# facebookresearch/vggsfm

Measured on NVIDIA H100. Metric: BA iterations/sec, higher is better.
Workload: dtype f64

## Files before the change

### vggsfm_b200/_lib.py

```python
from __future__ import annotations

import ctypes
import os

_HERE = os.path.dirname(os.path.abspath(__file__))
LIB_PATH = os.path.join(_HERE, "libvggsfm_b200.so")

EXPORTS = [
    "vgg_last_error", "vgg_version",
    "vgg_ba_default_options", "vgg_ba_dims", "vgg_ba_workspace_bytes", "vgg_ba_camrec_len",
    "vgg_ba_build_blocks", "vgg_ba_schur", "vgg_cholesky_lower", "vgg_ba_solve",
    "vgg_ba_reduced_system_doubles", "vgg_ba_fabric_doubles", "vgg_ba_solve_fabric",
    "vgg_ba_default_linear_solver", "vgg_ba_workspace_bytes_iterative", "vgg_ba_solve_iterative",
    "vgg_pose_default_options", "vgg_pose_refinement", "vgg_pnp_workspace_bytes", "vgg_absolute_pose_estimation", "vgg_syrk_ozaki_workspace_bytes", "vgg_syrk_ozaki",
    "vgg_tri_workspace_bytes", "vgg_triangulate_tracks", "vgg_triangulate_by_pair", "vgg_filter_points3d",
    "vgg_project_points", "vgg_normalize_tracks", "vgg_undistort_simple_radial",
    "vgg_corr_pyramid_bytes", "vgg_corr_build_pyramid", "vgg_corr_sample", "vgg_sample_features4d",
    "vgg_corr_tc_supported", "vgg_corr_tc_bytes", "vgg_corr_tc_build", "vgg_corr_tc_sample",
    "vgg_twoview_workspace_bytes", "vgg_estimate_fundamental", "vgg_relative_pose_from_fundamental",
    "vgg_fundamental_inliers", "vgg_msac_fundamental_workspace_bytes", "vgg_estimate_fundamental_msac",
    "vgg_depth_sparse_samples", "vgg_depth_median", "vgg_depth_ransac_workspace_bytes", "vgg_depth_ransac_max_chunk",
    "vgg_depth_ransac_begin", "vgg_depth_ransac_chunk", "vgg_depth_ransac_finish", "vgg_depth_tile_pixels",
    "vgg_depth_apply", "vgg_depth_unproject",
]


DEV_EXPORTS = ["vgg_dev_blocks_timing", "vgg_dev_blocks_last_ms", "vgg_dev_chol128_probe", "vgg_dev_syrk_f64", "vgg_dev_syrk_f64_band", "vgg_dev_trsv_probe", "vgg_dev_cholesky_band",
               "vgg_dev_last_band_hint", "vgg_dev_msac_trace", "vgg_dev_relative_pose_counts",
               "vgg_dev_build_blocks_band", "vgg_dev_schur_build", "vgg_dev_syrk_work_list", "vgg_dev_pcg_probe"]


class BAProblem(ctypes.Structure):
    _fields_ = [
        ("S", ctypes.c_int32), ("N", ctypes.c_int32),
        ("camera_model", ctypes.c_int32), ("intr_mode", ctypes.c_int32),
        ("uv", ctypes.c_void_p), ("mask", ctypes.c_void_p),
        ("param_const", ctypes.c_void_p), ("point_const", ctypes.c_void_p),
        ("poses", ctypes.c_void_p), ("intr", ctypes.c_void_p), ("points", ctypes.c_void_p),
        ("loss_function_type", ctypes.c_int32), ("loss_function_scale", ctypes.c_double),
    ]


class BAOptions(ctypes.Structure):
    _fields_ = [
        ("max_num_iterations", ctypes.c_int32),
        ("max_num_consecutive_invalid_steps", ctypes.c_int32),
        ("jacobi_scaling", ctypes.c_int32),
        ("reserved", ctypes.c_int32),
        ("function_tolerance", ctypes.c_double),
        ("gradient_tolerance", ctypes.c_double),
        ("parameter_tolerance", ctypes.c_double),
        ("initial_trust_region_radius", ctypes.c_double),
        ("max_trust_region_radius", ctypes.c_double),
        ("min_trust_region_radius", ctypes.c_double),
        ("min_relative_decrease", ctypes.c_double),
        ("min_lm_diagonal", ctypes.c_double),
        ("max_lm_diagonal", ctypes.c_double),
    ]


class BALinearSolver(ctypes.Structure):
    _fields_ = [
        ("type", ctypes.c_int32), ("min_linear_solver_iterations", ctypes.c_int32),
        ("max_linear_solver_iterations", ctypes.c_int32), ("eta", ctypes.c_double),
    ]


class BASummary(ctypes.Structure):
    _fields_ = [
        ("iterations", ctypes.c_int32), ("successful", ctypes.c_int32),
        ("termination", ctypes.c_int32), ("reserved", ctypes.c_int32),
        ("initial_cost", ctypes.c_double), ("final_cost", ctypes.c_double),
        ("final_radius", ctypes.c_double), ("device_ms", ctypes.c_double),
        ("kernel_launches", ctypes.c_int64),
    ]


class BAFabric(ctypes.Structure):
    _fields_ = [("ar_local", ctypes.c_void_p), ("ar_multicast", ctypes.c_void_p), ("ar_doubles", ctypes.c_size_t),
                ("world", ctypes.c_int32), ("rank", ctypes.c_int32), ("peer_base", ctypes.c_void_p * 8),
                ("total_doubles", ctypes.c_size_t)]


class PoseOptions(ctypes.Structure):
    _fields_ = [
        ("max_num_iterations", ctypes.c_int32),
        ("max_num_consecutive_invalid_steps", ctypes.c_int32),
        ("min_inliers", ctypes.c_int32),
        ("reserved", ctypes.c_int32),
        ("function_tolerance", ctypes.c_double),
        ("gradient_tolerance", ctypes.c_double),
        ("parameter_tolerance", ctypes.c_double),
        ("initial_trust_region_radius", ctypes.c_double),
        ("max_trust_region_radius", ctypes.c_double),
        ("min_trust_region_radius", ctypes.c_double),
        ("min_relative_decrease", ctypes.c_double),
        ("min_lm_diagonal", ctypes.c_double),
        ("max_lm_diagonal", ctypes.c_double),
        ("loss_function_scale", ctypes.c_double),
        ("max_reproj_error", ctypes.c_double),
    ]


ALLREDUCE_FN = ctypes.CFUNCTYPE(ctypes.c_int, ctypes.c_void_p, ctypes.c_void_p, ctypes.c_size_t,
                                ctypes.c_int, ctypes.c_void_p)

_lib = None


class NativeLibraryMissing(RuntimeError):
    pass


def lib() -> ctypes.CDLL:
    global _lib
    if _lib is not None:
        return _lib
    if not os.path.exists(LIB_PATH):
        raise NativeLibraryMissing(
            f"{LIB_PATH} not found: build it with `python -c 'import __graft_entry__ as g; g.build()'` "
            "or `make`. vggsfm_b200 has no CPU/PyTorch fallback.")
    L = ctypes.CDLL(LIB_PATH, mode=ctypes.RTLD_GLOBAL)
    L.vgg_last_error.restype = ctypes.c_char_p
    L.vgg_version.restype = ctypes.c_int
    L.vgg_ba_default_options.argtypes = [ctypes.POINTER(BAOptions)]
    L.vgg_ba_default_options.restype = None
    L.vgg_ba_dims.argtypes = [ctypes.c_int, ctypes.c_int, ctypes.POINTER(ctypes.c_int), ctypes.POINTER(ctypes.c_int)]
    L.vgg_ba_workspace_bytes.argtypes = [ctypes.c_int, ctypes.c_int, ctypes.c_int, ctypes.c_int,
                                         ctypes.POINTER(ctypes.c_size_t)]
    L.vgg_ba_camrec_len.argtypes = [ctypes.c_int, ctypes.c_int]
    L.vgg_ba_build_blocks.argtypes = [ctypes.POINTER(BAProblem)] + [ctypes.c_void_p] * 6 + [ctypes.c_int, ctypes.c_void_p]
    L.vgg_ba_schur.argtypes = ([ctypes.POINTER(BAProblem)] + [ctypes.c_void_p] * 5 +
                               [ctypes.c_double] * 3 + [ctypes.c_void_p, ctypes.c_size_t, ctypes.c_void_p,
                                                        ctypes.c_void_p, ctypes.POINTER(ctypes.c_int), ctypes.c_void_p])
    L.vgg_ba_solve.argtypes = [ctypes.POINTER(BAProblem), ctypes.POINTER(BAOptions), ctypes.c_void_p, ctypes.c_size_t,
                               ALLREDUCE_FN, ctypes.c_void_p, ctypes.POINTER(BASummary), ctypes.c_void_p,
                               ctypes.c_void_p]
    vp, ci, cd, cs = ctypes.c_void_p, ctypes.c_int, ctypes.c_double, ctypes.c_size_t
    L.vgg_ba_reduced_system_doubles.argtypes = [ci, ci, ci, ctypes.POINTER(cs)]
    L.vgg_ba_fabric_doubles.argtypes = [ci, ci, ci, ctypes.POINTER(cs)]
    L.vgg_ba_solve_fabric.argtypes = [ctypes.POINTER(BAProblem), ctypes.POINTER(BAOptions), vp, cs, ALLREDUCE_FN, vp,
                                      ctypes.POINTER(BAFabric), ctypes.POINTER(BASummary), vp, vp]
    L.vgg_ba_default_linear_solver.argtypes = [ctypes.POINTER(BALinearSolver)]
    L.vgg_ba_default_linear_solver.restype = None
    L.vgg_ba_workspace_bytes_iterative.argtypes = [ci, ci, ci, ci, ctypes.POINTER(cs)]
    L.vgg_ba_solve_iterative.argtypes = [ctypes.POINTER(BAProblem), ctypes.POINTER(BAOptions),
                                         ctypes.POINTER(BALinearSolver), vp, cs, ctypes.POINTER(BASummary), vp, vp, vp]
    L.vgg_dev_pcg_probe.argtypes = [ctypes.POINTER(BAProblem)] + [vp] * 6 + [cd] * 3 + [vp, vp, cs] + [vp] * 5
    L.vgg_pose_default_options.argtypes = [ctypes.POINTER(PoseOptions)]
    L.vgg_pose_default_options.restype = None
    L.vgg_pose_refinement.argtypes = [ci, ci, ci, vp, vp, vp, vp, vp, vp, ctypes.POINTER(PoseOptions), vp, vp, vp, vp]
    L.vgg_pnp_workspace_bytes.argtypes = [ci, ci, ctypes.POINTER(cs)]
    L.vgg_absolute_pose_estimation.argtypes = [ci, ci, ci, vp, vp, vp, vp, vp, vp, ci, ci, cd, vp, vp, vp, vp, vp, cs, vp]
    L.vgg_syrk_ozaki_workspace_bytes.argtypes = [ci, ci, ci, ctypes.POINTER(cs)]
    L.vgg_dev_blocks_timing.argtypes = [ci]
    L.vgg_dev_blocks_last_ms.argtypes = [ctypes.POINTER(cd)]
    L.vgg_dev_chol128_probe.argtypes = [ci, vp, vp, vp]
    L.vgg_dev_syrk_f64.argtypes = [ci, ci, vp, vp, vp]
    L.vgg_dev_syrk_f64_band.argtypes = L.vgg_dev_syrk_f64.argtypes + [vp, ci]
    L.vgg_dev_trsv_probe.argtypes = [ci, ci, vp, vp, cs, vp, vp]
    L.vgg_dev_last_band_hint.argtypes = [vp, vp, vp, vp, vp]
    L.vgg_dev_build_blocks_band.argtypes = L.vgg_ba_build_blocks.argtypes[:-1] + [vp, ci, vp]
    L.vgg_dev_schur_build.argtypes = [ctypes.POINTER(BAProblem)] + [vp] * 5 + [cd] * 3 + [ci, ci, vp, cs] + [vp] * 8
    L.vgg_dev_syrk_work_list.argtypes = [ci, ci, vp, ci, ci, vp, ci, ctypes.POINTER(ci)]
    L.vgg_syrk_ozaki.argtypes = [ci, ci, vp, vp, ci, vp, cs, vp]
    L.vgg_cholesky_lower.argtypes = [ci, ci, vp, vp, cs, ctypes.POINTER(ci), vp]
    L.vgg_dev_cholesky_band.argtypes = L.vgg_cholesky_lower.argtypes + [vp, ci, ci]
    L.vgg_tri_workspace_bytes.argtypes = [ci, ci, ci, ci, ctypes.POINTER(cs)]
    L.vgg_triangulate_tracks.argtypes = [ci, ci, vp, vp, vp, vp, vp, ci, ci, cd, cd, vp, vp, vp, vp, cs, vp]
    L.vgg_triangulate_by_pair.argtypes = [ci, ci, vp, vp, vp, vp, vp, vp, cs, vp]
    L.vgg_filter_points3d.argtypes = [ci, ci, vp, vp, ci, vp, vp, vp, cd, cd, ci, cd, vp, vp, vp, cs, vp]
    L.vgg_project_points.argtypes = [ci, ci, vp, vp, vp, vp, vp, vp, vp]
    L.vgg_normalize_tracks.argtypes = [ci, ci, vp, vp, vp, ci, vp, vp]
    L.vgg_undistort_simple_radial.argtypes = [ci, ci, vp, vp, ci, cd, cd, vp, ctypes.POINTER(ci), vp, cs, vp]
    L.vgg_corr_pyramid_bytes.argtypes = [ci, ci, ci, ci, ci, ci, ctypes.POINTER(cs), ctypes.POINTER(cs)]
    L.vgg_corr_build_pyramid.argtypes = [ci, ci, ci, ci, ci, vp, ci, vp, vp, vp]
    L.vgg_sample_features4d.argtypes = [ci, ci, ci, ci, ci, vp, vp, vp, vp]
    L.vgg_corr_sample.argtypes = [ci, ci, ci, ci, ci, ci, ci, vp, ci, vp, vp, ci, vp, vp]
    L.vgg_corr_tc_supported.argtypes = [ci, ci, ci, ci, ci]
    L.vgg_corr_tc_bytes.argtypes = [ci, ci, ci, ci, ci, ci, ctypes.POINTER(cs), ctypes.POINTER(cs)]
    L.vgg_corr_tc_build.argtypes = [ci, ci, ci, ci, ci, vp, vp, vp]
    L.vgg_corr_tc_sample.argtypes = [ci, ci, ci, ci, ci, ci, ci, vp, vp, vp, vp, vp, vp]
    L.vgg_twoview_workspace_bytes.argtypes = [ci, ci, ci, ci, ctypes.POINTER(cs)]
    L.vgg_estimate_fundamental.argtypes = [ci, ci, vp, vp, ci, vp, vp, ci, ci, cd, ci, ci, vp, vp, vp, vp, vp, cs, vp]
    L.vgg_fundamental_inliers.argtypes = [ci, ci, vp, vp, ci, vp, cd, ci, vp, vp]
    L.vgg_relative_pose_from_fundamental.argtypes = [ci, ci, vp, vp, ci, vp, cd, cd, vp, vp, vp, vp]
    L.vgg_dev_relative_pose_counts.argtypes = [ci, ci, vp, vp, ci, vp, cd, cd, vp, vp, vp, vp, vp]
    cu64 = ctypes.c_ulonglong
    L.vgg_msac_fundamental_workspace_bytes.argtypes = [ci, ci, ci, ci, ctypes.POINTER(cs)]
    L.vgg_estimate_fundamental_msac.argtypes = [ci, ci, vp, vp, ci, vp, cd, ci, ci, cu64, vp, vp, vp, vp, vp, cs, vp]
    L.vgg_dev_msac_trace.argtypes = [ci, ci, ci, ci, vp, ci, vp, vp, vp]
    i64 = ctypes.c_int64
    L.vgg_depth_sparse_samples.argtypes = [ci, vp, vp, cd, cd, vp, vp, vp, vp, vp, vp, vp]
    L.vgg_depth_median.argtypes = [ci, vp, vp, cd, vp, vp]
    L.vgg_depth_ransac_workspace_bytes.argtypes = [ci, ctypes.POINTER(cs)]
    L.vgg_depth_ransac_max_chunk.argtypes = []
    L.vgg_depth_ransac_begin.argtypes = [ci, ci, vp, cs, vp]
    L.vgg_depth_ransac_chunk.argtypes = [ci, vp, vp, vp, vp, ci, vp, ci, vp, vp, vp, cs, vp]
    L.vgg_depth_ransac_finish.argtypes = [ci, vp, vp, vp, vp, vp, vp, vp, vp, vp, vp, cs, vp]
    L.vgg_depth_tile_pixels.argtypes = []
    L.vgg_depth_apply.argtypes = [ci, i64, vp, vp, vp, vp, vp, vp, vp, vp]
    L.vgg_depth_unproject.argtypes = [ci, i64, vp, vp, vp, vp, vp, vp, vp, vp, vp, vp, vp, vp]
    _lib = L
    return L


def check(rc: int, what: str) -> None:
    if rc != 0:
        raise RuntimeError(f"{what} failed (rc={rc}): {lib().vgg_last_error().decode(errors='replace')}")
```

### vggsfm_b200/csrc/ba_schur.cu

```cuda
#include <stddef.h>
#include <algorithm>
#include <vector>
#include "ba_obs.h"
#include "common.cuh"
#include "dev_probes.h"
#include "syrk_work.h"

namespace vgg {

__device__ __forceinline__ void ar_add(double* local, double* mc, double v) {
  if (mc) asm volatile("multimem.red.relaxed.sys.global.add.f64 [%0], %1;" ::"l"(mc), "d"(v) : "memory");
  else atomicAdd(local, v);
}
__device__ __forceinline__ void ar_put(double* local, double* mc, double v) {
  if (mc) asm volatile("multimem.red.relaxed.sys.global.add.f64 [%0], %1;" ::"l"(mc), "d"(v) : "memory");
  else *local = v;
}

__global__ void jacobi_scale_points_kernel(int N, const double* __restrict__ H_pp, double* __restrict__ sc_p, int enable) {
  const int n = blockIdx.x * blockDim.x + threadIdx.x;
  if (n >= N) return;
  const double* h = H_pp + (size_t)n * 6;
  sc_p[n * 3 + 0] = enable ? 1.0 / (1.0 + sqrt(h[0])) : 1.0;
  sc_p[n * 3 + 1] = enable ? 1.0 / (1.0 + sqrt(h[3])) : 1.0;
// ... 154 lines not shown
    for (int i = 0; i < 4; ++i) pw[(12 + i) * 32 + lane] = frame_ok ? intr[(size_t)s * 4 + i] : 0.0;
    __syncwarp();
    double zq[DC];
#pragma unroll
    for (int i = 0; i < DC; ++i) zq[i] = 0.0;
    for (int t = 0; t < nt; ++t) {
      const size_t o = (size_t)s * N + n0 + t;
      const bool valid = frame_ok && mask[o] != 0;
      if (!__any_sync(0xffffffffu, valid)) continue;
      const float2 ob = frame_ok ? uv2[o] : make_float2(0.f, 0.f);
      const double* pt = s_pt[t];
      const double* m = pt + 4;
      double jc0[8], jc1[8], jx0[3], jx1[3], rx, ry, oc;
      obs_math<MODEL, ROBUST>(pw + lane, 32, pt[0], pt[1], pt[2], pt[3] != 0.0, ob.x, ob.y, valid, jc0, jc1, jx0, jx1,
                              rx, ry, loss, oc);
#pragma unroll
      for (int i = 0; i < DC; ++i) {
        const double w0 = w_entry(jc0, jc1, jx0, jx1, i, 0), w1 = w_entry(jc0, jc1, jx0, jx1, i, 1),
                     w2 = w_entry(jc0, jc1, jx0, jx1, i, 2);
        const double z0 = w0 * m[0];
        const double z1 = w0 * m[1] + w1 * m[4];
        const double z2 = w0 * m[2] + w1 * m[5] + w2 * m[8];
        zs[lane * DC + i] = z0;
        zs[ZR + lane * DC + i] = z1;
        zs[2 * ZR + lane * DC + i] = z2;
        zq[i] += z0 * m[9] + z1 * m[10] + z2 * m[11];
      }
      if (NS > 0) {
        double a[8];
#pragma unroll
        for (int k = 0; k < 8; ++k) a[k] = k < 3 * NS ? w_entry(jc0, jc1, jx0, jx1, 6 + k / 3, k % 3) : 0.0;
        const double r = warp_reduce_scatter<8>(a, lane);
        if (lane < 3 * NS) s_ws[warp][t][lane] += r;
      }
      __syncwarp();
      double* dst = Zt + (size_t)(3 * (n0 + t)) * Dpad + (size_t)g * ZR;
#pragma unroll
      for (int c = 0; c < 3; ++c, dst += Dpad) {
        const double* src = zs + c * ZR;
        for (int e = 2 * lane; e + 1 < cnt; e += 64)
          *reinterpret_cast<double2*>(dst + e) = *reinterpret_cast<const double2*>(src + e);
        if ((cnt & 1) && lane == 0) dst[cnt - 1] = src[cnt - 1];
      }
      __syncwarp();
    }
    if (frame_ok) {
#pragma unroll
      for (int i = 0; i < DC; ++i) {
        double* r = &rhs[(size_t)s * DC + i];
        if (zq[i] != 0.0) ar_add(r, mc_off ? r + mc_off : nullptr, zq[i]);
      }
    }
  }
  if (NS > 0) {
    __syncthreads();
    if ((int)threadIdx.x < nt * NS) {
      const int t = threadIdx.x / NS, j = threadIdx.x % NS;
      double w[3];
#pragma unroll
      for (int c = 0; c < 3; ++c) {
        w[c] = 0.0;
#pragma unroll
        for (int v = 0; v < ZB_W; ++v) w[c] += s_ws[v][t][j * 3 + c];
      }
      const double* m = s_pt[t] + 4;
      const double z0 = w[0] * m[0];
      const double z1 = w[0] * m[1] + w[1] * m[4];
      const double z2 = w[0] * m[2] + w[1] * m[5] + w[2] * m[8];
      double* zo = Zt + (size_t)(3 * (n0 + t)) * Dpad + (size_t)S * DC + j;
      zo[0] = z0;
      zo[Dpad] = z1;
      zo[2 * (size_t)Dpad] = z2;
      const double zq = z0 * m[9] + z1 * m[10] + z2 * m[11];
      double* r = &rhs[(size_t)S * DC + j];
      if (zq != 0.0) ar_add(r, mc_off ? r + mc_off : nullptr, zq);
    }
  }
}

constexpr int SF_BM = 128, SF_BK = 16, SF_LDS = 132, SF_STAGES = 4, SF_MMA_WARPS = 8;
constexpr int SF_THREADS = 128 + SF_MMA_WARPS * 32;
constexpr int SF_STAGE_DOUBLES = 2 * SF_BK * SF_LDS;
constexpr size_t SF_SMEM_BYTES = sizeof(double) * SF_STAGES * SF_STAGE_DOUBLES + sizeof(uint64_t) * 2 * SF_STAGES;

struct SyrkWork {
  int bi, bj, kb0, kb1;
};

__global__ void __launch_bounds__(SF_THREADS, 1)
    syrk_f64_kernel(const SyrkWork* __restrict__ work, int nwork, int Kpad, int Dpad, const double* __restrict__ Zt,
                    double* __restrict__ Cmat, ptrdiff_t mc_off, const __grid_constant__ FabricDev fd) {
  extern __shared__ __align__(16) double sf_smem[];
  uint64_t* full = reinterpret_cast<uint64_t*>(sf_smem + SF_STAGES * SF_STAGE_DOUBLES);
  uint64_t* empty = full + SF_STAGES;
  const int warp = threadIdx.x >> 5, lane = threadIdx.x & 31;
  if (threadIdx.x == 0) {
    for (int s = 0; s < SF_STAGES; ++s) {
      mbar_init(&full[s], 1);
      mbar_init(&empty[s], SF_MMA_WARPS);
    }
    mbar_fence_init();
  }
  __syncthreads();

  int stage = 0, phase = 0;
  if (warp < 4) {
    asm volatile("setmaxnreg.dec.sync.aligned.u32 40;");
    if (warp > 0) return;
    const int row = lane & (SF_BK - 1), opnd = lane / SF_BK;
    for (int w = blockIdx.x; w < nwork; w += gridDim.x) {
      const SyrkWork wk = work[w];
      const bool diag = wk.bi == wk.bj;
      const int k1 = min(Kpad, wk.kb1 * 64);
      for (int k = wk.kb0 * 64; k < k1; k += SF_BK) {
        mbar_wait(&empty[stage], phase ^ 1);
        if (lane == 0) mbar_expect_tx(&full[stage], (diag ? 1u : 2u) * SF_BK * SF_BM * (uint32_t)sizeof(double));
        __syncwarp();
        if (opnd == 0 || !diag)
          tma_load_1d(sf_smem + stage * SF_STAGE_DOUBLES + (opnd * SF_BK + row) * SF_LDS,
                      Zt + (size_t)(k + row) * Dpad + (opnd ? wk.bj : wk.bi) * SF_BM, SF_BM * sizeof(double), &full[stage]);
        if (++stage == SF_STAGES) {
          stage = 0;
          phase ^= 1;
        }
      }
    }
    return;
  }

  asm volatile("setmaxnreg.inc.sync.aligned.u32 232;");
  const int wm = (warp - 4) >> 2, wn = warp & 3;
  const int g = lane >> 2, t = lane & 3;
  for (int w = blockIdx.x; w < nwork; w += gridDim.x) {
    const SyrkWork wk = work[w];
    const bool diag = wk.bi == wk.bj;
    const int k1 = min(Kpad, wk.kb1 * 64);
    double acc[4][4][4];
#pragma unroll
    for (int mt = 0; mt < 4; ++mt)
#pragma unroll
      for (int nt = 0; nt < 4; ++nt)
#pragma unroll
        for (int h = 0; h < 4; ++h) acc[mt][nt][h] = 0.0;
    for (int k = wk.kb0 * 64; k < k1; k += SF_BK) {
      mbar_wait(&full[stage], phase);
      const double* as = sf_smem + stage * SF_STAGE_DOUBLES + t * SF_LDS + wm * 64 + g;
      const double* bs = sf_smem + stage * SF_STAGE_DOUBLES + (diag ? 0 : SF_BK * SF_LDS) + t * SF_LDS + wn * 32 + g;
      double b[4][4];
#pragma unroll
      for (int nt = 0; nt < 4; ++nt)
#pragma unroll
        for (int j = 0; j < 4; ++j) b[nt][j] = bs[4 * j * SF_LDS + nt * 8];
#pragma unroll
      for (int mt = 0; mt < 4; ++mt) {
        double a[8];
#pragma unroll
        for (int i = 0; i < 8; ++i) a[i] = as[4 * (i >> 1) * SF_LDS + mt * 16 + 8 * (i & 1)];
#pragma unroll
        for (int nt = 0; nt < 4; ++nt) dmma_m16n8k16(acc[mt][nt], a, b[nt]);
      }
      __syncwarp();
      if (lane == 0) mbar_arrive(&empty[stage]);
      if (++stage == SF_STAGES) {
        stage = 0;
        phase ^= 1;
      }
    }
#pragma unroll
    for (int mt = 0; mt < 4; ++mt)
#pragma unroll
      for (int nt = 0; nt < 4; ++nt)
#pragma unroll
        for (int h = 0; h < 4; ++h) {
          const int r = wk.bi * SF_BM + wm * 64 + mt * 16 + g + 8 * (h >> 1);
          const int col = wk.bj * SF_BM + wn * 32 + nt * 8 + 2 * t + (h & 1);
          syrk_red_upper(Cmat, Dpad, r, col, wk.bj, diag, acc[mt][nt][h], mc_off, fd);
        }
  }
}

__global__ void scale_damp_kernel(int D, int Dpad, double* __restrict__ A, const double* __restrict__ rhs,
                                  const double* __restrict__ hdiag, const double* __restrict__ sc,
                                  const uint8_t* __restrict__ pconst, double radius, double min_diag, double max_diag,
                                  double* __restrict__ bvec) {
  const int j = blockIdx.x * blockDim.x + threadIdx.x;
  const int i = blockIdx.y;
  if (j >= D || j > i) return;
  const bool ci = pconst[i] != 0, cj = pconst[j] != 0;
  double v;
  if (ci || cj) {
    v = (i == j) ? 1.0 : 0.0;
  } else {
    v = A[(size_t)i * Dpad + j] * sc[i] * sc[j];
    if (i == j) v += fmin(fmax(hdiag[i] * sc[i] * sc[i], min_diag), max_diag) / radius;
  }
  A[(size_t)i * Dpad + j] = v;
  if (i == j) {
    const double b = ci ? 0.0 : rhs[i] * sc[i];
    bvec[i] = b;
    A[(size_t)D * Dpad + i] = b;
    if (i == 0) A[(size_t)D * Dpad + D] = 1e300;
  }
}

__global__ void cam_step_kernel(int D, const double* __restrict__ dcs, size_t dcs_stride, const double* __restrict__ sc,
                                const double* __restrict__ hdiag, const double* __restrict__ gvec,
                                const uint8_t* __restrict__ pconst, double radius, double min_diag, double max_diag,
                                double* __restrict__ d_c, double* __restrict__ scal) {
  const int i = blockIdx.x * blockDim.x + threadIdx.x;
  double a = 0, b = 0, bad = 0;
  if (i < D) {
    const double x = pconst[i] ? 0.0 : dcs[(size_t)i * dcs_stride];
    const double dc = x * sc[i];
    d_c[i] = dc;
    if (!isfinite(x)) bad = 1.0;
    const double dcc = fmin(fmax(hdiag[i] * sc[i] * sc[i], min_diag), max_diag);
    a = pconst[i] ? 0.0 : (x * x * dcc / radius - dc * gvec[i]);
    b = dc * dc;
  }
  a = warp_sum(a); b = warp_sum(b); bad = warp_sum(bad);
  if ((threadIdx.x & 31) == 0) {
    atomicAdd(&scal[0], a);
    atomicAdd(&scal[1], b);
    if (bad > 0) atomicAdd(&scal[7], bad);
  }
}

constexpr int BS_W = 16;
template <int MODEL, int MODE, bool ROBUST>
__global__ void __launch_bounds__(BS_W * 32) backsub_kernel(
    int S, int N, const float* __restrict__ uv, const uint8_t* __restrict__ mask, const double* __restrict__ poses,
    const double* __restrict__ intr, const double* __restrict__ points, const uint8_t* __restrict__ point_const,
    const double* __restrict__ d_c, double* __restrict__ wacc, const int* __restrict__ fg_tracks, BaLoss loss) {
  using C = BlkCfg<MODEL, MODE>;
  constexpr int DC = C::DC, NS = C::NS;
  __shared__ double s_cam[BS_W][16];
  __shared__ double s_acc[3][BS_W][32];
  const int lane = threadIdx.x & 31, warp = threadIdx.x >> 5, nw = blockDim.x >> 5;
  const int nlo = blockIdx.x * 32, nhi = min(N, nlo + 32);
  const int n = nlo + lane;
  const bool track_ok = n < N;
  double X0 = 0.0, X1 = 0.0, X2 = 0.0;
  bool pc = true;
  if (track_ok) {
    X0 = points[(size_t)n * 3]; X1 = points[(size_t)n * 3 + 1]; X2 = points[(size_t)n * 3 + 2];
    pc = point_const && point_const[n] != 0;
  }
  double dsh[2] = {0.0, 0.0};
#pragma unroll
  for (int j = 0; j < NS; ++j) dsh[j] = d_c[(size_t)S * DC + j];
  const float2* uv2 = reinterpret_cast<const float2*>(uv);
  double* cam = s_cam[warp];
  double w0 = 0.0, w1 = 0.0, w2 = 0.0;
  for (int s = warp; s < S; s += nw) {
    if (fg_tracks && (nhi <= fg_tracks[2 * (s >> 5)] || nlo >= fg_tracks[2 * (s >> 5) + 1])) continue;
    const size_t o = (size_t)s * N + n;
    const bool valid = track_ok && mask[o] != 0;
    if (!__any_sync(0xffffffffu, valid)) continue;
    const float2 ob = valid ? uv2[o] : make_float2(0.f, 0.f);
    __syncwarp();
// ... 114 lines not shown
  if (i >= D) return;
  gvec[i] = (i < S * dc) ? camrec[(size_t)(i / dc) * KR + (i % dc)] : shared_in[i - S * dc];
}

__global__ void gradmax_kernel(int D, int N, const double* __restrict__ gvec, const uint8_t* __restrict__ pconst,
                               const double* __restrict__ g_p, const uint8_t* __restrict__ point_const,
                               double* __restrict__ scal) {
  const int i = blockIdx.x * blockDim.x + threadIdx.x;
  unsigned long long mc = 0, mp = 0;
  if (i < D && !pconst[i]) mc = (unsigned long long)__double_as_longlong(fabs(gvec[i]));
  if (i < N * 3 && !(point_const && point_const[i / 3])) mp = (unsigned long long)__double_as_longlong(fabs(g_p[i]));
#pragma unroll
  for (int off = 16; off >= 1; off >>= 1) {
    mc = max(mc, __shfl_xor_sync(0xffffffffu, mc, off));
    mp = max(mp, __shfl_xor_sync(0xffffffffu, mp, off));
  }
  if ((threadIdx.x & 31) == 0) {
    atomicMax(reinterpret_cast<unsigned long long*>(&scal[4]), mc);
    atomicMax(reinterpret_cast<unsigned long long*>(&scal[5]), mp);
  }
}

int launch_jacobi_scale_points(int N, const double* H_pp, double* sc_p, int enable, cudaStream_t st) {
  jacobi_scale_points_kernel<<<(N + 255) / 256, 256, 0, st>>>(N, H_pp, sc_p, enable);
  VGG_LAUNCH_CHECK();
  return VGG_OK;
}
int launch_jacobi_scale_cams(int D, const double* hdiag, double* sc_c, int enable, cudaStream_t st) {
  jacobi_scale_cams_kernel<<<(D + 255) / 256, 256, 0, st>>>(D, hdiag, sc_c, enable);
  VGG_LAUNCH_CHECK();
  return VGG_OK;
}
int launch_point_prep(int N, const double* H_pp, const double* g_p, const double* sc_p, const uint8_t* point_const,
                      double radius, double min_diag, double max_diag, double* M, double* q, double* dpp,
                      double* scal, cudaStream_t st) {
  point_prep_kernel<<<(N + 127) / 128, 128, 0, st>>>(N, H_pp, g_p, sc_p, point_const, radius, min_diag, max_diag, M, q,
                                                     dpp, scal);
  VGG_LAUNCH_CHECK();
  return VGG_OK;
}
int launch_assemble_hc(int S, int dc, int ns, int KR, int Dpad, const double* camrec, const double* shared_in,
                       double* Sraw, double* rhs, double* hdiag, double* gvec, ptrdiff_t mc_off, cudaStream_t st) {
  assemble_hc_kernel<<<S + (ns > 0 ? 1 : 0), 64, 0, st>>>(S, dc, ns, KR, Dpad, camrec, shared_in, Sraw, rhs, hdiag, gvec,
                                                          mc_off);
  VGG_LAUNCH_CHECK();
  return VGG_OK;
}
#define VGG_PICK_BA_KERNEL(kern, tmpl, p)                                                          \
  decltype(&tmpl<0, 0, false>) kern = nullptr;                                                      \
  {                                                                                                 \
    const bool robust = (p)->loss_function_type != VGG_LOSS_TRIVIAL;                               \
    switch ((p)->camera_model * 3 + (p)->intr_mode) {                                               \
      case 0: kern = robust ? tmpl<0, 0, true> : tmpl<0, 0, false>; break;                           \
      case 1: kern = robust ? tmpl<0, 1, true> : tmpl<0, 1, false>; break;                           \
      case 2: kern = robust ? tmpl<0, 2, true> : tmpl<0, 2, false>; break;                           \
      case 3: kern = robust ? tmpl<1, 0, true> : tmpl<1, 0, false>; break;                           \
      case 4: kern = robust ? tmpl<1, 1, true> : tmpl<1, 1, false>; break;                           \
      case 5: kern = robust ? tmpl<1, 2, true> : tmpl<1, 2, false>; break;                           \
    }                                                                                               \
  }                                                                                                 \
  VGG_REQUIRE(kern, "bad camera_model/intr_mode")

int launch_z_build(const vgg_ba_problem* p, int Dpad, const double* M, const double* q, double* Zt, double* rhs,
                   ptrdiff_t mc_off, const int* fg_tracks, cudaStream_t st) {
  VGG_PICK_BA_KERNEL(kern, z_build_kernel, p);
  const int nw = std::min(ZB_W, (p->S + 31) / 32);
  kern<<<(p->N + ZB_NT - 1) / ZB_NT, nw * 32, 0, st>>>(p->S, p->N, Dpad, p->uv, p->mask, p->poses, p->intr, p->points,
                                                        p->point_const, M, q, Zt, rhs, mc_off, fg_tracks, ba_loss_of(p));
  VGG_LAUNCH_CHECK();
  return VGG_OK;
}

struct SyrkF64State {
  int dev = -1, Kpad = -1, Dpad = -1, sms = 0, nwork = 0;
  std::vector<int> ranges;
  SyrkWork* work_dev = nullptr;
  size_t work_cap = 0;
};
thread_local SyrkF64State g_sf;

static std::vector<SyrkWork> syrk_f64_work(int Kpad, int Dpad, const std::vector<int>& ranges, int nworkers) {
  const int nb = Dpad / SF_BM, KB = (Kpad + 63) / 64;
  std::vector<SyrkWork> work;
  build_work_list<SyrkWork>({1}, syrk_tile_jobs(nb, ranges), KB, nworkers, KB, 1,
                            [](const SyrkTileJob& j, int, int k0, int k1) { return SyrkWork{j.bi, j.bj, k0, k1}; }, &work);
  return work;
}

int launch_syrk(int Kpad, int Dpad, const double* Zt, double* Cmat, ptrdiff_t mc_off, const std::vector<int>& kb_ranges,
                const FabricDev& fd, cudaStream_t st) {
  VGG_REQUIRE(Dpad % SF_BM == 0 && Kpad % SF_BK == 0, "syrk: Dpad must be a multiple of 128 and Kpad of 16");
  const int nb = Dpad / SF_BM;
  SyrkF64State& hs = g_sf;
  const std::vector<int> ranges = (int)kb_ranges.size() == 2 * nb ? kb_ranges : std::vector<int>();
  int dev = 0;
  VGG_CUDA_CHECK(cudaGetDevice(&dev));
  if (hs.dev != dev || hs.Kpad != Kpad || hs.Dpad != Dpad || hs.ranges != ranges) {
    VGG_CUDA_CHECK(cudaDeviceGetAttribute(&hs.sms, cudaDevAttrMultiProcessorCount, dev));
    VGG_CUDA_CHECK(cudaFuncSetAttribute(syrk_f64_kernel, cudaFuncAttributeMaxDynamicSharedMemorySize, (int)SF_SMEM_BYTES));
    const std::vector<SyrkWork> work = syrk_f64_work(Kpad, Dpad, ranges, hs.sms);
    VGG_CUDA_CHECK(cudaDeviceSynchronize());
    if (hs.dev != dev || work.size() > hs.work_cap) {
      if (hs.work_dev) cudaFree(hs.work_dev);
      hs.work_dev = nullptr;
      hs.work_cap = std::max<size_t>(work.size(), 1);
      VGG_CUDA_CHECK(cudaMalloc(reinterpret_cast<void**>(&hs.work_dev), sizeof(SyrkWork) * hs.work_cap));
    }
    if (!work.empty())
      VGG_CUDA_CHECK(cudaMemcpy(hs.work_dev, work.data(), sizeof(SyrkWork) * work.size(), cudaMemcpyHostToDevice));
    hs.nwork = (int)work.size();
    hs.dev = dev;
    hs.Kpad = Kpad;
    hs.Dpad = Dpad;
    hs.ranges = ranges;
  }
  if (hs.nwork == 0) return VGG_OK;
  syrk_f64_kernel<<<std::min(hs.sms, hs.nwork), SF_THREADS, SF_SMEM_BYTES, st>>>(hs.work_dev, hs.nwork, Kpad, Dpad, Zt, Cmat,
                                                                               mc_off, fd);
  VGG_LAUNCH_CHECK();
  return VGG_OK;
}
int launch_scale_damp(int D, int Dpad, double* A, const double* rhs, const double* hdiag, const double* sc,
                      const uint8_t* pconst, double radius, double min_diag, double max_diag, double* bvec,
                      cudaStream_t st) {
  dim3 grid((D + 255) / 256, D);
  scale_damp_kernel<<<grid, 256, 0, st>>>(D, Dpad, A, rhs, hdiag, sc, pconst, radius, min_diag, max_diag, bvec);
  VGG_LAUNCH_CHECK();
  return VGG_OK;
}
int launch_cam_step(int D, const double* dcs, size_t dcs_stride, const double* sc, const double* hdiag, const double* gvec,
                    const uint8_t* pconst, double radius, double min_diag, double max_diag, double* d_c, double* scal,
                    cudaStream_t st) {
  cam_step_kernel<<<(D + 255) / 256, 256, 0, st>>>(D, dcs, dcs_stride, sc, hdiag, gvec, pconst, radius, min_diag, max_diag, d_c, scal);
  VGG_LAUNCH_CHECK();
  return VGG_OK;
}
int launch_backsub(const vgg_ba_problem* p, const double* d_c, double* wacc, const int* fg_tracks, cudaStream_t st) {
  VGG_PICK_BA_KERNEL(kern, backsub_kernel, p);
  const int nw = std::min(BS_W, p->S);
  kern<<<(p->N + 31) / 32, nw * 32, 0, st>>>(p->S, p->N, p->uv, p->mask, p->poses, p->intr, p->points, p->point_const,
                                             d_c, wacc, fg_tracks, ba_loss_of(p));
  VGG_LAUNCH_CHECK();
  return VGG_OK;
}
int launch_point_step(int N, const double* M, const double* g_p, const double* wacc, const double* sc_p,
                      const double* dpp, const uint8_t* point_const, const double* X, double radius, double* Xc,
                      double* scal, cudaStream_t st) {
  point_step_kernel<<<(N + 127) / 128, 128, 0, st>>>(N, M, g_p, wacc, sc_p, dpp, point_const, X, radius, Xc, scal);
  VGG_LAUNCH_CHECK();
  return VGG_OK;
}
int launch_cam_update(int S, int dc, int ns, int model, const double* d_c, const double* poses, const double* intr,
                      double* poses_c, double* intr_c, cudaStream_t st) {
  cam_update_kernel<<<(S + 127) / 128, 128, 0, st>>>(S, dc, ns, model, d_c, poses, intr, poses_c, intr_c);
  VGG_LAUNCH_CHECK();
  return VGG_OK;
}
int launch_extract_gvec(int S, int dc, int ns, int KR, const double* camrec, const double* shared_in, double* gvec,
                        cudaStream_t st) {
  const int D = S * dc + ns;
  extract_gvec_kernel<<<(D + 255) / 256, 256, 0, st>>>(S, dc, ns, KR, camrec, shared_in, gvec);
  VGG_LAUNCH_CHECK();
  return VGG_OK;
}
int launch_gradmax(int D, int N, const double* gvec, const uint8_t* pconst, const double* g_p,
                   const uint8_t* point_const, double* scal, cudaStream_t st) {
  const int n = D > N * 3 ? D : N * 3;
  gradmax_kernel<<<(n + 255) / 256, 256, 0, st>>>(D, N, gvec, pconst, g_p, point_const, scal);
  VGG_LAUNCH_CHECK();
  return VGG_OK;
}

}

extern "C" {

int vgg_dev_syrk_f64(int Kpad, int Dpad, const double* Zt, double* Cmat, void* stream) {
  return vgg_dev_syrk_f64_band(Kpad, Dpad, Zt, Cmat, stream, nullptr, 0);
}

int vgg_dev_syrk_f64_band(int Kpad, int Dpad, const double* Zt, double* Cmat, void* stream, const int* ranges, int count) {
  using namespace vgg;
  g_launch_count = 0;
  VGG_REQUIRE(Zt && Cmat && Kpad > 0 && Dpad > 0 && (ranges || count <= 0), "bad argument");
  return launch_syrk(Kpad, Dpad, Zt, Cmat, 0, std::vector<int>(ranges, ranges + std::max(count, 0)), FabricDev{},
                     static_cast<cudaStream_t>(stream));
}

int vgg_dev_syrk_work_list(int Kpad, int Dpad, const int* ranges, int count, int nworkers, int* items, int cap,
                           int* nwork) {
  using namespace vgg;
  VGG_REQUIRE(Kpad > 0 && Kpad % SF_BK == 0 && Dpad > 0 && Dpad % SF_BM == 0 && nworkers > 0 && nwork &&
                  (ranges || count <= 0),
              "bad argument");
  std::vector<int> r(ranges, ranges + std::max(count, 0));
  if ((int)r.size() != 2 * (Dpad / SF_BM)) r.clear();
  const std::vector<SyrkWork> work = syrk_f64_work(Kpad, Dpad, r, nworkers);
  *nwork = (int)work.size();
  if (!items) return VGG_OK;
  VGG_REQUIRE((int)work.size() <= cap, "work list longer than cap");
  for (size_t i = 0; i < work.size(); ++i) {
    items[4 * i] = work[i].bi;
    items[4 * i + 1] = work[i].bj;
    items[4 * i + 2] = work[i].kb0;
    items[4 * i + 3] = work[i].kb1;
  }
  return VGG_OK;
}

}
```

### vggsfm_b200/csrc/dev_probes.h

```cpp
#pragma once
#ifdef __cplusplus
extern "C" {
#endif
int vgg_dev_blocks_timing(int enable);
int vgg_dev_blocks_last_ms(double* ms);
int vgg_dev_chol128_probe(int reps, const double* A_host, double* L_host, long long* prof13_host);
int vgg_dev_syrk_f64(int Kpad, int Dpad, const double* Zt, double* Cmat, void* stream);
int vgg_dev_syrk_f64_band(int Kpad, int Dpad, const double* Zt, double* Cmat, void* stream, const int* ranges_host,
                          int count);
int vgg_dev_trsv_probe(int n, int lda, const double* A_dev, const double* y_dev, size_t y_stride, double* x_dev,
                       long long* stamps_host);
int vgg_dev_last_band_hint(int* meta_host, int* rb_range, int* end_blk, int* kb_rows, int* fg_tracks);
int vgg_dev_cholesky_band(int n, int lda, double* A, void* workspace, size_t ws_bytes, int* info_host, void* stream,
                          const int* end_blk_host, int count, int arrow_blk);
int vgg_dev_msac_trace(int B, int N, int max_iterations, int min_iterations, const void* workspace, int cap,
                       int32_t* lo_runs_host, int32_t* win_trial_host, int32_t* lo_trials_host);
int vgg_dev_relative_pose_counts(int B, int N, const void* points1, const void* points2, int points_are_f64,
                                 const double* fmat, double width, double height, double* R_out, double* t_out,
                                 double* E_out, int32_t* counts_dev, void* stream);

int vgg_dev_build_blocks_band(const vgg_ba_problem* prob, double* cost, double* camrec, double* g_p, double* H_pp,
                              double* W, double* shared, int tracks_per_warp, const int* fg_tracks_host, int count,
                              void* stream);
int vgg_dev_schur_build(const vgg_ba_problem* prob, const double* camrec, const double* g_p, const double* H_pp,
                        const double* shared, const double* scale_p, double radius, double min_diag, double max_diag,
                        int banded, int zt_nan, void* workspace, size_t ws_bytes, double* M, double* q, double* dpp,
                        double* scal, double* Zt, double* Sraw, double* rhs, void* stream);
int vgg_dev_syrk_work_list(int Kpad, int Dpad, const int* ranges_host, int count, int nworkers, int* items_host,
                           int cap, int* nwork);

int vgg_dev_pcg_probe(const vgg_ba_problem* prob, const double* camrec, const double* g_p, const double* H_pp,
                      const double* shared_in, const double* scale_p, const double* scale_c, double radius,
                      double min_diag, double max_diag, const double* x_in, void* workspace, size_t ws_bytes,
                      double* y_out, double* b_out, double* pinv_out, double* state_out, void* stream);

#ifdef __cplusplus
}
#endif
```

### vggsfm_b200/csrc/syrk_work.h

```cpp
#pragma once
#include <algorithm>
#include <utility>
#include <vector>

namespace vgg {

struct SyrkTileJob {
  int bi, bj;
  int kb0 = 0, kb1 = -1;
};

inline std::vector<SyrkTileJob> syrk_tile_jobs(int nb, const std::vector<int>& ranges) {
  const bool banded = (int)ranges.size() == 2 * nb;
  std::vector<SyrkTileJob> jobs;
  for (int bi = 0; bi < nb; ++bi)
    for (int bj = 0; bj <= bi; ++bj) {
      SyrkTileJob jb{bj, bi};
      if (banded) {
        jb.kb0 = std::max(ranges[2 * bi], ranges[2 * bj]);
        jb.kb1 = std::min(ranges[2 * bi + 1], ranges[2 * bj + 1]);
        if (jb.kb1 <= jb.kb0) continue;
      }
      jobs.push_back(jb);
    }
  return jobs;
}

template <class Work, class Make>
void build_work_list(const std::vector<int>& group_cost, const std::vector<SyrkTileJob>& jobs, int KB, int nworkers,
                     int max_item_kb, long long epilogue_cost, Make make, std::vector<Work>* out) {
  long long total = 0, cost_all = 0;
  for (int c : group_cost) cost_all += c;
  for (const SyrkTileJob& jb : jobs) total += cost_all * (long long)((jb.kb1 < 0 ? KB : jb.kb1) - jb.kb0);
  long long best = -1;
  for (int div = 2; div <= 10; ++div) {
    const long long target = std::max<long long>(1, total / ((long long)nworkers * div));
    std::vector<std::pair<long long, Work>> items;
    for (const SyrkTileJob& jb : jobs) {
      const int jk0 = jb.kb0, jk1 = jb.kb1 < 0 ? KB : jb.kb1, len = jk1 - jk0;
      if (len <= 0) continue;
      for (int g = 0; g < (int)group_cost.size(); ++g) {
        const long long cost = (long long)group_cost[g] * len;
        int parts = (int)std::min<long long>(16, std::max<long long>(1, (cost + target / 2) / target));
        parts = std::max(parts, (len + max_item_kb - 1) / max_item_kb);
        parts = std::min(parts, len);
        for (int p = 0; p < parts; ++p) {
          const int k0 = jk0 + (int)((long long)len * p / parts), k1 = jk0 + (int)((long long)len * (p + 1) / parts);
          items.push_back({(long long)group_cost[g] * (k1 - k0), make(jb, g, k0, k1)});
        }
      }
    }
    std::stable_sort(items.begin(), items.end(), [](const auto& a, const auto& b) { return a.first > b.first; });
    std::vector<long long> load(nworkers, 0);
    for (size_t i = 0; i < items.size(); ++i) load[i % nworkers] += items[i].first + epilogue_cost;
    const long long makespan = *std::max_element(load.begin(), load.end());
    if (best < 0 || makespan < best) {
      best = makespan;
      out->clear();
      for (auto& it : items) out->push_back(it.second);
    }
  }
}

}
```

Baseline: 374.7.

## Specialize diagonal SYRK tiles and rebalance work list with per-tile costs

Diagonal tiles of the f64 SYRK now take a dedicated path. Eight MMA warps split only the upper-triangular 9 n-tiles per row pair, so the redundant lower-triangle MMAs that the square tile path computed on diagonal blocks are skipped. The host work-list builder is replaced by a balanced scheduler that costs diagonal and off-diagonal tiles differently and searches over how many jobs stay whole and the split granularity. A templated probe variant with globaltimer/clock stamps is also added for diagnostics but is not used on the default path.

```diff
diff --git a/vggsfm_b200/_lib.py b/vggsfm_b200/_lib.py
--- a/vggsfm_b200/_lib.py
+++ b/vggsfm_b200/_lib.py
@@ -25,7 +25,7 @@
 ]
 
 
-DEV_EXPORTS = ["vgg_dev_blocks_timing", "vgg_dev_blocks_last_ms", "vgg_dev_chol128_probe", "vgg_dev_syrk_f64", "vgg_dev_syrk_f64_band", "vgg_dev_trsv_probe", "vgg_dev_cholesky_band",
+DEV_EXPORTS = ["vgg_dev_blocks_timing", "vgg_dev_blocks_last_ms", "vgg_dev_chol128_probe", "vgg_dev_syrk_f64", "vgg_dev_syrk_f64_band", "vgg_dev_syrk_f64_probe", "vgg_dev_trsv_probe", "vgg_dev_cholesky_band",
                "vgg_dev_last_band_hint", "vgg_dev_msac_trace", "vgg_dev_relative_pose_counts",
                "vgg_dev_build_blocks_band", "vgg_dev_schur_build", "vgg_dev_syrk_work_list", "vgg_dev_pcg_probe"]
 
@@ -158,6 +158,7 @@
     L.vgg_dev_chol128_probe.argtypes = [ci, vp, vp, vp]
     L.vgg_dev_syrk_f64.argtypes = [ci, ci, vp, vp, vp]
     L.vgg_dev_syrk_f64_band.argtypes = L.vgg_dev_syrk_f64.argtypes + [vp, ci]
+    L.vgg_dev_syrk_f64_probe.argtypes = L.vgg_dev_syrk_f64.argtypes + [vp, ci, ctypes.POINTER(ci)]
     L.vgg_dev_trsv_probe.argtypes = [ci, ci, vp, vp, cs, vp, vp]
     L.vgg_dev_last_band_hint.argtypes = [vp, vp, vp, vp, vp]
     L.vgg_dev_build_blocks_band.argtypes = L.vgg_ba_build_blocks.argtypes[:-1] + [vp, ci, vp]
diff --git a/vggsfm_b200/csrc/ba_schur.cu b/vggsfm_b200/csrc/ba_schur.cu
--- a/vggsfm_b200/csrc/ba_schur.cu
+++ b/vggsfm_b200/csrc/ba_schur.cu
@@ -260,18 +260,69 @@
 constexpr int SF_THREADS = 128 + SF_MMA_WARPS * 32;
 constexpr int SF_STAGE_DOUBLES = 2 * SF_BK * SF_LDS;
 constexpr size_t SF_SMEM_BYTES = sizeof(double) * SF_STAGES * SF_STAGE_DOUBLES + sizeof(uint64_t) * 2 * SF_STAGES;
+constexpr int SF_PROBE_ITEMS = 16, SF_PROBE_REC = 8 + 4 * SF_PROBE_ITEMS;
+constexpr int SF_COST_OFF = 16, SF_COST_DIAG = 10, SF_COST_EPILOGUE = 16;
 
 struct SyrkWork {
   int bi, bj, kb0, kb1;
 };
 
+__device__ __forceinline__ long long sf_globaltimer() {
+  long long t;
+  asm volatile("mov.u64 %0, %%globaltimer;" : "=l"(t));
+  return t;
+}
+
+template <int SPLIT, bool PROBE>
+__device__ __forceinline__ long long sf_diag_steps(double (&acc)[9][4], const double* smem, uint64_t* full,
+                                                   uint64_t* empty, int& stage, int& phase, int nsteps, int r0, int r1,
+                                                   int n0, int n1, int lane) {
+  const int g = lane >> 2, t = lane & 3;
+  long long waited = 0;
+  for (int step = 0; step < nsteps; ++step) {
+    long long c0 = 0;
+    if (PROBE) c0 = clock64();
+    mbar_wait(&full[stage], phase);
+    if (PROBE) waited += clock64() - c0;
+    const double* s = smem + stage * SF_STAGE_DOUBLES + t * SF_LDS + g;
+    double a0[8], a1[8];
+#pragma unroll
+    for (int i = 0; i < 8; ++i) a0[i] = s[4 * (i >> 1) * SF_LDS + r0 * 16 + 8 * (i & 1)];
+    if (SPLIT < 9) {
+#pragma unroll
+      for (int i = 0; i < 8; ++i) a1[i] = s[4 * (i >> 1) * SF_LDS + r1 * 16 + 8 * (i & 1)];
+    }
+#pragma unroll
+    for (int j = 0; j < 9; ++j) {
+      double b[4];
+#pragma unroll
+      for (int i = 0; i < 4; ++i) b[i] = s[4 * i * SF_LDS + ((j < SPLIT ? n0 : n1) + j) * 8];
+      dmma_m16n8k16(acc[j], j < SPLIT ? a0 : a1, b);
+    }
+    __syncwarp();
+    if (lane == 0) mbar_arrive(&empty[stage]);
+    if (++stage == SF_STAGES) {
+      stage = 0;
+      phase ^= 1;
+    }
+  }
+  return waited;
+}
+
+template <bool PROBE>
 __global__ void __launch_bounds__(SF_THREADS, 1)
     syrk_f64_kernel(const SyrkWork* __restrict__ work, int nwork, int Kpad, int Dpad, const double* __restrict__ Zt,
-                    double* __restrict__ Cmat, ptrdiff_t mc_off, const __grid_constant__ FabricDev fd) {
+                    double* __restrict__ Cmat, ptrdiff_t mc_off, const __grid_constant__ FabricDev fd,
+                    long long* __restrict__ probe) {
   extern __shared__ __align__(16) double sf_smem[];
   uint64_t* full = reinterpret_cast<uint64_t*>(sf_smem + SF_STAGES * SF_STAGE_DOUBLES);
   uint64_t* empty = full + SF_STAGES;
   const int warp = threadIdx.x >> 5, lane = threadIdx.x & 31;
+  long long* prec = PROBE ? probe + (size_t)blockIdx.x * SF_PROBE_REC : nullptr;
+  if (PROBE && threadIdx.x == 0) {
+    prec[0] = sf_globaltimer();
+    prec[1] = clock64();
+  }
   if (threadIdx.x == 0) {
     for (int s = 0; s < SF_STAGES; ++s) {
       mbar_init(&full[s], 1);
@@ -309,10 +360,50 @@
   asm volatile("setmaxnreg.inc.sync.aligned.u32 232;");
   const int wm = (warp - 4) >> 2, wn = warp & 3;
   const int g = lane >> 2, t = lane & 3;
-  for (int w = blockIdx.x; w < nwork; w += gridDim.x) {
+  const int dpair = (warp - 4) >> 1, dsecond = warp & 1;
+  const int ds = dsecond ? 7 - 2 * dpair : 9, dr0 = dpair, dr1 = 7 - dpair;
+  const int dn0 = dsecond ? 2 * dpair + 9 : 2 * dpair, dn1 = 14 - 2 * dpair - ds;
+  long long wait_cycles = 0, ksteps = 0;
+  int item = 0;
+  for (int w = blockIdx.x; w < nwork; w += gridDim.x, ++item) {
     const SyrkWork wk = work[w];
     const bool diag = wk.bi == wk.bj;
     const int k1 = min(Kpad, wk.kb1 * 64);
+    if (PROBE && warp == 4 && lane == 0 && item < SF_PROBE_ITEMS) {
+      prec[8 + 4 * item] = sf_globaltimer();
+      prec[11 + 4 * item] = w;
+    }
+    if (diag) {
+      double acc[9][4];
+#pragma unroll
+      for (int j = 0; j < 9; ++j)
+#pragma unroll
+        for (int h = 0; h < 4; ++h) acc[j][h] = 0.0;
+      const int nsteps = (k1 - wk.kb0 * 64 + SF_BK - 1) / SF_BK;
+      long long waited = 0;
+      switch (ds) {
+        case 9: waited = sf_diag_steps<9, PROBE>(acc, sf_smem, full, empty, stage, phase, nsteps, dr0, dr1, dn0, dn1, lane); break;
+        case 7: waited = sf_diag_steps<7, PROBE>(acc, sf_smem, full, empty, stage, phase, nsteps, dr0, dr1, dn0, dn1, lane); break;
+        case 5: waited = sf_diag_steps<5, PROBE>(acc, sf_smem, full, empty, stage, phase, nsteps, dr0, dr1, dn0, dn1, lane); break;
+        case 3: waited = sf_diag_steps<3, PROBE>(acc, sf_smem, full, empty, stage, phase, nsteps, dr0, dr1, dn0, dn1, lane); break;
+        default: waited = sf_diag_steps<1, PROBE>(acc, sf_smem, full, empty, stage, phase, nsteps, dr0, dr1, dn0, dn1, lane);
+      }
+      if (PROBE) {
+        wait_cycles += waited;
+        ksteps += nsteps;
+        if (lane == 0 && item < SF_PROBE_ITEMS) atomicMax(&prec[9 + 4 * item], sf_globaltimer());
+      }
+#pragma unroll
+      for (int j = 0; j < 9; ++j)
+#pragma unroll
+        for (int h = 0; h < 4; ++h) {
+          const int r = wk.bi * SF_BM + (j < ds ? dr0 : dr1) * 16 + g + 8 * (h >> 1);
+          const int col = wk.bj * SF_BM + ((j < ds ? dn0 : dn1) + j) * 8 + 2 * t + (h & 1);
+          syrk_red_upper(Cmat, Dpad, r, col, wk.bj, true, acc[j][h], mc_off, fd);
+        }
+      if (PROBE && lane == 0 && item < SF_PROBE_ITEMS) atomicMax(&prec[10 + 4 * item], sf_globaltimer());
+      continue;
+    }
     double acc[4][4][4];
 #pragma unroll
     for (int mt = 0; mt < 4; ++mt)
@@ -321,9 +412,15 @@
 #pragma unroll
         for (int h = 0; h < 4; ++h) acc[mt][nt][h] = 0.0;
     for (int k = wk.kb0 * 64; k < k1; k += SF_BK) {
+      long long c0 = 0;
+      if (PROBE) c0 = clock64();
       mbar_wait(&full[stage], phase);
+      if (PROBE) {
+        wait_cycles += clock64() - c0;
+        ++ksteps;
+      }
       const double* as = sf_smem + stage * SF_STAGE_DOUBLES + t * SF_LDS + wm * 64 + g;
-      const double* bs = sf_smem + stage * SF_STAGE_DOUBLES + (diag ? 0 : SF_BK * SF_LDS) + t * SF_LDS + wn * 32 + g;
+      const double* bs = sf_smem + stage * SF_STAGE_DOUBLES + SF_BK * SF_LDS + t * SF_LDS + wn * 32 + g;
       double b[4][4];
 #pragma unroll
       for (int nt = 0; nt < 4; ++nt)
@@ -344,6 +441,7 @@
         phase ^= 1;
       }
     }
+    if (PROBE && lane == 0 && item < SF_PROBE_ITEMS) atomicMax(&prec[9 + 4 * item], sf_globaltimer());
 #pragma unroll
     for (int mt = 0; mt < 4; ++mt)
 #pragma unroll
@@ -352,8 +450,18 @@
         for (int h = 0; h < 4; ++h) {
           const int r = wk.bi * SF_BM + wm * 64 + mt * 16 + g + 8 * (h >> 1);
           const int col = wk.bj * SF_BM + wn * 32 + nt * 8 + 2 * t + (h & 1);
-          syrk_red_upper(Cmat, Dpad, r, col, wk.bj, diag, acc[mt][nt][h], mc_off, fd);
+          syrk_red_upper(Cmat, Dpad, r, col, wk.bj, false, acc[mt][nt][h], mc_off, fd);
         }
+    if (PROBE && lane == 0 && item < SF_PROBE_ITEMS) atomicMax(&prec[10 + 4 * item], sf_globaltimer());
+  }
+  if (PROBE && lane == 0) {
+    atomicAdd(reinterpret_cast<unsigned long long*>(&prec[4]), (unsigned long long)wait_cycles);
+    atomicMax(&prec[2], (long long)clock64());
+    atomicMax(&prec[3], sf_globaltimer());
+    if (warp == 4) {
+      prec[5] = ksteps;
+      prec[6] = item;
+    }
   }
 }
 
@@ -634,13 +742,15 @@
 static std::vector<SyrkWork> syrk_f64_work(int Kpad, int Dpad, const std::vector<int>& ranges, int nworkers) {
   const int nb = Dpad / SF_BM, KB = (Kpad + 63) / 64;
   std::vector<SyrkWork> work;
-  build_work_list<SyrkWork>({1}, syrk_tile_jobs(nb, ranges), KB, nworkers, KB, 1,
-                            [](const SyrkTileJob& j, int, int k0, int k1) { return SyrkWork{j.bi, j.bj, k0, k1}; }, &work);
+  build_balanced_work_list<SyrkWork>(syrk_tile_jobs(nb, ranges), KB, nworkers, SF_COST_OFF, SF_COST_DIAG,
+                                     SF_COST_EPILOGUE,
+                                     [](const SyrkTileJob& j, int k0, int k1) { return SyrkWork{j.bi, j.bj, k0, k1}; },
+                                     &work);
   return work;
 }
 
-int launch_syrk(int Kpad, int Dpad, const double* Zt, double* Cmat, ptrdiff_t mc_off, const std::vector<int>& kb_ranges,
-                const FabricDev& fd, cudaStream_t st) {
+static int syrk_launch(int Kpad, int Dpad, const double* Zt, double* Cmat, ptrdiff_t mc_off,
+                       const std::vector<int>& kb_ranges, const FabricDev& fd, cudaStream_t st, long long* probe) {
   VGG_REQUIRE(Dpad % SF_BM == 0 && Kpad % SF_BK == 0, "syrk: Dpad must be a multiple of 128 and Kpad of 16");
   const int nb = Dpad / SF_BM;
   SyrkF64State& hs = g_sf;
@@ -649,7 +759,10 @@
   VGG_CUDA_CHECK(cudaGetDevice(&dev));
   if (hs.dev != dev || hs.Kpad != Kpad || hs.Dpad != Dpad || hs.ranges != ranges) {
     VGG_CUDA_CHECK(cudaDeviceGetAttribute(&hs.sms, cudaDevAttrMultiProcessorCount, dev));
-    VGG_CUDA_CHECK(cudaFuncSetAttribute(syrk_f64_kernel, cudaFuncAttributeMaxDynamicSharedMemorySize, (int)SF_SMEM_BYTES));
+    VGG_CUDA_CHECK(cudaFuncSetAttribute(syrk_f64_kernel<false>, cudaFuncAttributeMaxDynamicSharedMemorySize,
+                                        (int)SF_SMEM_BYTES));
+    VGG_CUDA_CHECK(cudaFuncSetAttribute(syrk_f64_kernel<true>, cudaFuncAttributeMaxDynamicSharedMemorySize,
+                                        (int)SF_SMEM_BYTES));
     const std::vector<SyrkWork> work = syrk_f64_work(Kpad, Dpad, ranges, hs.sms);
     VGG_CUDA_CHECK(cudaDeviceSynchronize());
     if (hs.dev != dev || work.size() > hs.work_cap) {
@@ -667,10 +780,15 @@
     hs.ranges = ranges;
   }
   if (hs.nwork == 0) return VGG_OK;
-  syrk_f64_kernel<<<std::min(hs.sms, hs.nwork), SF_THREADS, SF_SMEM_BYTES, st>>>(hs.work_dev, hs.nwork, Kpad, Dpad, Zt, Cmat,
-                                                                               mc_off, fd);
-  VGG_LAUNCH_CHECK();
-  return VGG_OK;
+  auto kern = probe ? syrk_f64_kernel<true> : syrk_f64_kernel<false>;
+  kern<<<std::min(hs.sms, hs.nwork), SF_THREADS, SF_SMEM_BYTES, st>>>(hs.work_dev, hs.nwork, Kpad, Dpad, Zt, Cmat, mc_off,
+                                                                     fd, probe);
+  VGG_LAUNCH_CHECK();
+  return VGG_OK;
+}
+int launch_syrk(int Kpad, int Dpad, const double* Zt, double* Cmat, ptrdiff_t mc_off, const std::vector<int>& kb_ranges,
+                const FabricDev& fd, cudaStream_t st) {
+  return syrk_launch(Kpad, Dpad, Zt, Cmat, mc_off, kb_ranges, fd, st, nullptr);
 }
 int launch_scale_damp(int D, int Dpad, double* A, const double* rhs, const double* hdiag, const double* sc,
                       const uint8_t* pconst, double radius, double min_diag, double max_diag, double* bvec,
@@ -737,6 +855,22 @@
   VGG_REQUIRE(Zt && Cmat && Kpad > 0 && Dpad > 0 && (ranges || count <= 0), "bad argument");
   return launch_syrk(Kpad, Dpad, Zt, Cmat, 0, std::vector<int>(ranges, ranges + std::max(count, 0)), FabricDev{},
                      static_cast<cudaStream_t>(stream));
+}
+
+int vgg_dev_syrk_f64_probe(int Kpad, int Dpad, const double* Zt, double* Cmat, void* stream, long long* stamps,
+                           int cap, int* nctas) {
+  using namespace vgg;
+  g_launch_count = 0;
+  VGG_REQUIRE(Zt && Cmat && stamps && nctas && Kpad > 0 && Dpad > 0, "bad argument");
+  int dev = 0, sms = 0;
+  VGG_CUDA_CHECK(cudaGetDevice(&dev));
+  VGG_CUDA_CHECK(cudaDeviceGetAttribute(&sms, cudaDevAttrMultiProcessorCount, dev));
+  const int n = std::min<int>(sms, (int)syrk_f64_work(Kpad, Dpad, {}, sms).size());
+  *nctas = n;
+  VGG_REQUIRE(cap >= n * SF_PROBE_REC, "stamps buffer shorter than nctas * record");
+  cudaStream_t st = static_cast<cudaStream_t>(stream);
+  VGG_CUDA_CHECK(cudaMemsetAsync(stamps, 0, sizeof(long long) * n * SF_PROBE_REC, st));
+  return syrk_launch(Kpad, Dpad, Zt, Cmat, 0, {}, FabricDev{}, st, stamps);
 }
 
 int vgg_dev_syrk_work_list(int Kpad, int Dpad, const int* ranges, int count, int nworkers, int* items, int cap,
diff --git a/vggsfm_b200/csrc/dev_probes.h b/vggsfm_b200/csrc/dev_probes.h
--- a/vggsfm_b200/csrc/dev_probes.h
+++ b/vggsfm_b200/csrc/dev_probes.h
@@ -8,6 +8,8 @@
 int vgg_dev_syrk_f64(int Kpad, int Dpad, const double* Zt, double* Cmat, void* stream);
 int vgg_dev_syrk_f64_band(int Kpad, int Dpad, const double* Zt, double* Cmat, void* stream, const int* ranges_host,
                           int count);
+int vgg_dev_syrk_f64_probe(int Kpad, int Dpad, const double* Zt, double* Cmat, void* stream, long long* stamps_dev,
+                           int cap, int* nctas);
 int vgg_dev_trsv_probe(int n, int lda, const double* A_dev, const double* y_dev, size_t y_stride, double* x_dev,
                        long long* stamps_host);
 int vgg_dev_last_band_hint(int* meta_host, int* rb_range, int* end_blk, int* kb_rows, int* fg_tracks);
diff --git a/vggsfm_b200/csrc/syrk_work.h b/vggsfm_b200/csrc/syrk_work.h
--- a/vggsfm_b200/csrc/syrk_work.h
+++ b/vggsfm_b200/csrc/syrk_work.h
@@ -62,4 +62,59 @@
   }
 }
 
+template <class Work, class Make>
+long long build_balanced_work_list(const std::vector<SyrkTileJob>& jobs, int KB, int nworkers, int off_cost,
+                                   int diag_cost, long long epilogue_cost, Make make, std::vector<Work>* out) {
+  struct Job {
+    int k0, len;
+    long long cost;
+    const SyrkTileJob* jb;
+  };
+  std::vector<Job> js;
+  long long total = 0;
+  for (const SyrkTileJob& jb : jobs) {
+    const int k0 = jb.kb0, len = (jb.kb1 < 0 ? KB : jb.kb1) - jb.kb0;
+    if (len <= 0) continue;
+    js.push_back({k0, len, (long long)(jb.bi == jb.bj ? diag_cost : off_cost) * len, &jb});
+    total += js.back().cost;
+  }
+  std::stable_sort(js.begin(), js.end(), [](const Job& a, const Job& b) { return a.cost > b.cost; });
+  const int nj = (int)js.size();
+  std::vector<int> wholes{0};
+  for (int n = std::max(1, nworkers - 16); n <= std::min(nj - 1, nworkers + 16); ++n) wholes.push_back(n);
+  struct Item {
+    int len;
+    long long cost;
+    int job, k0, k1;
+  };
+  std::vector<Item> items, best_items;
+  std::vector<long long> load(nworkers);
+  long long best = -1;
+  for (int whole : wholes)
+    for (int x4 = 4; x4 <= 48; ++x4) {
+      const long long target = std::max<long long>(1, total * 4 / ((long long)nworkers * x4));
+      items.clear();
+      for (int j = 0; j < nj; ++j) {
+        const Job& jb = js[j];
+        int parts = j < whole ? 1 : (int)std::min<long long>(16, std::max<long long>(1, (jb.cost + target / 2) / target));
+        parts = std::min(parts, jb.len);
+        for (int p = 0; p < parts; ++p) {
+          const int k0 = jb.k0 + (int)((long long)jb.len * p / parts), k1 = jb.k0 + (int)((long long)jb.len * (p + 1) / parts);
+          items.push_back({k1 - k0, jb.cost / jb.len * (k1 - k0), j, k0, k1});
+        }
+      }
+      std::stable_sort(items.begin(), items.end(), [](const Item& a, const Item& b) { return a.len > b.len; });
+      std::fill(load.begin(), load.end(), 0);
+      for (size_t i = 0; i < items.size(); ++i) load[i % nworkers] += items[i].cost + epilogue_cost;
+      const long long makespan = *std::max_element(load.begin(), load.end());
+      if (best < 0 || makespan < best) {
+        best = makespan;
+        best_items = items;
+      }
+    }
+  out->clear();
+  for (const Item& it : best_items) out->push_back(make(*js[it.job].jb, it.k0, it.k1));
+  return best;
 }
+
+}
```

New measurement: 381.7, median of 6. 1.9% higher.
